# lucidrains/nuwa-pytorch

Hardware: AMD Instinct MI355X
Metric: video-tokens/sec, 3DNA decoder fwd+bwd @ 10x16x16 (higher is better)
Workload: dtype bf16/fp16 operands, fp32 accumulate -- forward: 3-MFMA bf16 hi+lo pairs on cross-attention kv projection, to_logits; 2 fp16 MFMAs (fp16 activation x fp16 hi+lo weight) on to_out x2, cross-attention q projection; single fp16 MFMA on 3DNA q/k/v projection, FF1 + gate, FF2, Sparse3DNA core, cross-atten

## Files before the change

nuwa_pytorch_amd/csrc/s3_args.h:

```cpp
#pragma once
#include "common.h"
#include "../../include/amdnuwa.h"

struct S3Args {
    const bf16_t *q, *k, *v, *ql, *kl, *vl; int ld;
    bf16_t *o, *ol; int ldo;
    int ol_f16;
    const bf16_t *dO, *dOl; int lddo;
    bf16_t *dq, *dk, *dv, *dql, *dkl, *dvl; int ldd;
    const float* wth;
    const float* bias;
    float *ds, *pm;
    float* stats;
    float *part_th, *part_k0, *part_v0;
    float* dwth;
    int B, ntok, F, H, W, kf, kh, kw, df, dh, dw, NH;
    int of, oh, ow;
    int xmode, FK, kvrows, kvoff, ldk, lddk;
    const bf16_t *k0, *k0l, *v0, *v0l; long long k0_bs;
    const uint8_t* kmask;
    float *dnull_k, *dnull_v;
    float scale;
    int accumulate;
    int dbg;
    int ymajor;
    int sep_passes;
    int packed;
    const float* gs2;
    int NT, TW, SW;
};

struct S3DropArgs : S3Args { const uint8_t* keep; float drop_s; };
template <bool DROP> struct S3KArgsSel { using type = S3Args; };
template <> struct S3KArgsSel<true> { using type = S3DropArgs; };
template <bool DROP> using S3KArgs = typename S3KArgsSel<DROP>::type;
template <bool DROP> inline S3KArgs<DROP> s3_kargs(const S3Args& a, const uint8_t* keep, float drop_s) {
    if constexpr (DROP) {
        S3DropArgs d{};
        static_cast<S3Args&>(d) = a;
        d.keep = keep; d.drop_s = drop_s;
        return d;
    } else {
        return a;
    }
}

struct S3Tile { int tw, nt, sw; };
inline S3Tile s3_tile(const amdnuwa_s3_geom* g) {
    if (g->W * g->heads * 4 <= 512) return {g->W, 1, g->W};
    const int twmax = 128 / g->heads, nt = (g->W + twmax - 1) / twmax, tw = (g->W + nt - 1) / nt;
    long long halo = (long long)(g->kw - 1) * g->dw;
    if (halo > 65536) halo = 65536;
    return {tw, nt, tw + (int)halo};
}
int s3w_fwd_launch(const S3Args& a, int dim_head, bool lo, size_t lds, const uint8_t* keep, float drop_s, hipStream_t stream);
int s3w_bwd_launch(const S3Args& a, int dim_head, bool lo, size_t lds_q, size_t lds_kv, const uint8_t* keep, float drop_s, hipStream_t stream);

namespace {

template <bool F16> __device__ __forceinline__ float ld16_t(bf16_t v) { return F16 ? (float)__builtin_bit_cast(_Float16, v) : bf2f(v); }

constexpr float NEG_MAX = -3.4028234663852886e38f;

__device__ __forceinline__ int xcd_row_id() {
    const int nb = gridDim.x, id = blockIdx.x, per = nb >> 3, rem = nb & 7, x = id & 7, k = id >> 3;
    return x * per + (x < rem ? x : rem) + k;
}
// ... 75 lines not shown
```

nuwa_pytorch_amd/csrc/sparse3dna.hip:

```cpp
#include <cmath>
#include "common.h"
#include "s3_args.h"

namespace {

constexpr int KHMAX = 3;

struct PlaneIt { int ta, tb, fr, yr; };

template <int CH, typename Fn>
__device__ __forceinline__ void sweep_taps(const S3Args& a, const bf16_t* src, const bf16_t* srcl, int b, int f, int y, int w,
                                           int h, int c, bool act, bool qvalid, bf16_t* st_hi, Fn&& fn) {
    const int HS = a.W * a.NH * 32;
    bf16_t* st_lo = st_hi + (CH / 8) * HS;
    const int myslot = ((w * a.NH + h) * 4 + c) * 8;
    const int yr0 = y - a.oh * a.dh;
    uint4 rh[CH / 8], rl[CH / 8];
    auto seek = [&](PlaneIt& p) {
        while (p.ta < a.kf && !(p.fr >= 0 && p.yr >= 0 && p.fr < a.FK && p.yr < a.H)) {
            ++p.tb; p.yr += a.dh;
            if (p.tb == a.kh) { p.tb = 0; p.yr = yr0; ++p.ta; p.fr += a.df; }
        }
    };
    auto step = [&](PlaneIt& p) {
// ... 468 lines not shown
                *reinterpret_cast<uint4*>(sq_hi + myslot + v8 * HS) = rq[v8];
                *reinterpret_cast<uint4*>(sd_hi + myslot + v8 * HS) = rd[v8];
                if (a.ql) *reinterpret_cast<uint4*>(sq_lo + myslot + v8 * HS) = rql[v8];
                if (a.dOl) *reinterpret_cast<uint4*>(sd_lo + myslot + v8 * HS) = rdl[v8];
            }
        }
        __syncthreads();
        float cds[KWMAX], cpm[KWMAX];
#pragma unroll
        for (int tc = 0; tc < KWMAX; ++tc) { cds[tc] = nds[tc]; cpm[tc] = npm[tc]; }
        const int tn = next_plane(tp + 1);
        if (tn < nplanes) fetch(tn);
        if (kvalid) {
            int fq, yq;
            plane(tp, fq, yq);
            for (int tc = 0; tc < a.kw; ++tc) {
                const int wq = w + (a.ow - tc) * a.dw;
                if (wq < 0 || wq >= a.W) continue;
                const int pq = (fq * a.H + yq) * a.W + wq;
                if (1 + pq >= a.ntok) continue;
                float dsv, pmv;
                if (tc < KWMAX) { dsv = tc == 0 ? cds[0] : (tc == 1 ? cds[1] : cds[2]); pmv = tc == 0 ? cpm[0] : (tc == 1 ? cpm[1] : cpm[2]); }
                else {
                    const size_t ci = (((size_t)b * nq + pq) * J + 1 + slot_plane(tp) * a.kw + tc) * a.NH + h;
                    dsv = a.ds[ci]; pmv = a.pm[ci];
                }
                const int slot = ((wq * a.NH + h) * 4 + c) * 8;
                if (LO) {
                    float qq[CH], dd[CH];
                    load_chunk<CH>(sq_hi + slot, a.ql ? sq_lo + slot : nullptr, qq, HS);
                    load_chunk<CH>(sd_hi + slot, a.dOl ? sd_lo + slot : nullptr, dd, HS);
#pragma unroll
                    for (int e = 0; e < CH; ++e) { dkf[e] += dsv * qq[e]; dvf[e] += pmv * dd[e]; }
                } else {
                    uint32_t qk2[CH / 2], dk2[CH / 2];
                    load_pk<CH>(sq_hi + slot, qk2, HS);
                    load_pk<CH>(sd_hi + slot, dk2, HS);
                    axpy_pk<CH>(dkf, dsv, qk2);
                    axpy_pk<CH>(dvf, pmv, dk2);
                }
            }
        }
        tp = tn;
    }
    if (kvalid) {
#pragma unroll
        for (int e = 0; e < CH; ++e) dkf[e] *= a.scale;
        const size_t g = ((size_t)b * a.kvrows + ik) * a.lddk + h * DH + c * CH;
        store_chunk<CH>(a.dk + g, a.dkl ? a.dkl + g : nullptr, dkf);
        store_chunk<CH>(a.dv + g, a.dvl ? a.dvl + g : nullptr, dvf);
    }
}

__global__ __launch_bounds__(1024) void s3_bwd_fin_kernel(S3Args a, int DH) {
    __shared__ float red[2][16][64];
    const int rows = a.F * a.H * a.NT, inner = a.NH * DH;
    const int lane = threadIdx.x & 63, rg = threadIdx.x >> 6;
    const int nchunk = (inner + 63) / 64;
    if ((int)blockIdx.x >= a.B * nchunk) {
        __shared__ float redw[64][17];
        const int nn = a.NH * a.NH;
        const int col = (blockIdx.x - a.B * nchunk) * 16 + (threadIdx.x & 15), rg64 = threadIdx.x >> 4;
        float s = 0.f;
        if (col < nn) {
            const int n = a.B * rows;
            for (int k = rg64; k < n; k += 64 * 8) {
                float v[8];
#pragma unroll
                for (int u = 0; u < 8; ++u) {
                    const int ku = k + 64 * u;
                    const float t = a.part_th[(size_t)(ku < n ? ku : 0) * nn + col];
                    v[u] = ku < n ? t : 0.f;
                }
#pragma unroll
                for (int u = 0; u < 8; ++u) s += v[u];
            }
        }
        redw[rg64][threadIdx.x & 15] = s;
        __syncthreads();
        if (rg64 == 0 && col < nn) {
            float t = 0.f;
#pragma unroll
            for (int r = 0; r < 64; ++r) t += redw[r][threadIdx.x & 15];
            t *= f16_gs_inv(a.gs2);
            a.dwth[col] = a.accumulate ? a.dwth[col] + t : t;
        }
        return;
    }
    if (a.xmode) {
        if ((int)blockIdx.x >= nchunk) return;
        const int e = blockIdx.x * 64 + lane;
        float sk = 0.f, sv = 0.f;
        if (e < inner)
            for (int r = rg; r < a.B * rows; r += 16) {
                sk += a.part_k0[(size_t)r * inner + e];
                sv += a.part_v0[(size_t)r * inner + e];
            }
        red[0][rg][lane] = sk;
        red[1][rg][lane] = sv;
        __syncthreads();
        if (rg == 0 && e < inner) {
            float tk = 0.f, tv = 0.f;
#pragma unroll
            for (int r = 0; r < 16; ++r) { tk += red[0][r][lane]; tv += red[1][r][lane]; }
            a.dnull_k[e] = tk;
            a.dnull_v[e] = tv;
        }
        return;
    }
    const int b = blockIdx.x / nchunk, e = (blockIdx.x % nchunk) * 64 + lane;
    float sk = 0.f, sv = 0.f;
    if (e < inner)
        for (int r = rg; r < rows; r += 16 * 4) {
            float vk[4], vv[4];
#pragma unroll
            for (int u = 0; u < 4; ++u) {
                const int ru = r + 16 * u;
                const size_t o = ((size_t)b * rows + (ru < rows ? ru : 0)) * inner + e;
                const float tk = a.part_k0[o], tv = a.part_v0[o];
                vk[u] = ru < rows ? tk : 0.f; vv[u] = ru < rows ? tv : 0.f;
            }
#pragma unroll
            for (int u = 0; u < 4; ++u) { sk += vk[u]; sv += vv[u]; }
        }
    red[0][rg][lane] = sk;
    red[1][rg][lane] = sv;
    __syncthreads();
    if (rg == 0 && e < inner) {
        float tk = 0.f, tv = 0.f;
#pragma unroll
        for (int r = 0; r < 16; ++r) { tk += red[0][r][lane]; tv += red[1][r][lane]; }
        const size_t gi = ((size_t)b * a.ntok) * a.lddo + e, go = ((size_t)b * a.ntok) * a.ldd + e;
        if (a.gs2) {
            tv += ld16_t<true>(a.dO[gi]);
            float amax = fmaxf(fabsf(tk), fabsf(tv));
            a.dk[go] = f2h_sat(tk); a.dv[go] = f2h_sat(tv);
            f16_sat_commit(amax);
            return;
        }
        tv += bf2f(a.dO[gi]) + (a.dOl ? bf2f(a.dOl[gi]) : 0.f);
        bf16_t hh, ll;
        f2bf_hilo(tk, hh, ll); a.dk[go] = hh; if (a.dkl) a.dkl[go] = ll;
        f2bf_hilo(tv, hh, ll); a.dv[go] = hh; if (a.dvl) a.dvl[go] = ll;
    }
}

int check_geom(const amdnuwa_s3_geom* g) {
    if (!g) return AMDNUWA_ERR_ARG;
    if (g->dim_head != 32 && g->dim_head != 64) return AMDNUWA_ERR_UNSUPPORTED;
    if (g->heads < 1 || g->heads > 8 || g->W < 1 || (g->W * g->heads * 4 > 512 && g->W > 64)) return AMDNUWA_ERR_UNSUPPORTED;
    if (g->kf < 1 || g->kh < 1 || g->kw < 1 || g->df < 1 || g->dh < 1 || g->dw < 1) return AMDNUWA_ERR_ARG;
    if (g->ntok < 1 || g->ntok - 1 > g->F * g->H * g->W) return AMDNUWA_ERR_ARG;
    return AMDNUWA_OK;
}
constexpr size_t S3_LDS_MAX = 160 * 1024 - 2048;
struct S3Lds { size_t fwd, bq, bkv; };
S3Lds s3_lds(const amdnuwa_s3_geom* g, bool lo) {
    const S3Tile tl = s3_tile(g);
    const size_t J = (size_t)g->kf * g->kh * g->kw + 1, inner = (size_t)g->heads * g->dim_head, tw = (size_t)tl.tw, sw = (size_t)tl.sw;
    const size_t stage = sw * inner * (lo ? 4 : 2), nsp = tw * J * g->heads;
    size_t spdp = 2 * nsp;
    if (spdp < tw * inner) spdp = tw * inner;
    return {stage + nsp * 4, stage + (spdp + 8 * 64) * 4, sw * inner * 8};
}
size_t s3_lds_need(const amdnuwa_s3_geom* g, bool lo) {
    const S3Lds l = s3_lds(g, lo);
    const size_t m = l.fwd > l.bq ? l.fwd : l.bq;
    return m > l.bkv ? m : l.bkv;
}
typedef __attribute__((address_space(3))) s16x4 lds_s16x4_t;
__device__ __forceinline__ int vt_off(int row, int gc) { return row * 128 + ((gc ^ (row & 7)) << 4); }
__device__ __forceinline__ bf16x8 vt_tr(const char* tile, int db, int c, int g4) {
    const int col = db * 16 + ((c & 3) << 2);
    const int r0 = 4 * g4 + (c >> 2), r1 = 16 + r0;
    const s16x4 lo = __builtin_amdgcn_ds_read_tr16_b64_v4i16((lds_s16x4_t*)(tile + vt_off(r0, col >> 3) + ((col >> 2) & 1) * 8));
    const s16x4 hi = __builtin_amdgcn_ds_read_tr16_b64_v4i16((lds_s16x4_t*)(tile + vt_off(r1, col >> 3) + ((col >> 2) & 1) * 8));
// ... 1025 lines not shown
#pragma unroll
            for (int i = 0; i < ROWS; ++i)
#pragma unroll
                for (int db = 0; db < 4; ++db) O[i][db] = f32x4{0.f, 0.f, 0.f, 0.f};
        }
#pragma unroll
        for (int i = 0; i < ROWS; ++i) {
            if (!r.qok[i]) continue;
            const size_t go = (r.tok0 + r.iq[i]) * a.ldo + g * DH + 4 * r.g4;
#pragma unroll
            for (int db = 0; db < 4; ++db) {
                const uint32_t h01 = pack2_rne(O[i][db][0], O[i][db][1]), h23 = pack2_rne(O[i][db][2], O[i][db][3]);
                if (!F16 || a.o) *reinterpret_cast<uint2*>(a.o + go + db * 16) = make_uint2(h01, h23);
                if (F16 && a.ol)
                    *reinterpret_cast<uint2*>(a.ol + go + db * 16) = a.ol_f16 ?
                        make_uint2(pack2_f16_sat(O[i][db][0], O[i][db][1]), pack2_f16_sat(O[i][db][2], O[i][db][3])) :
                        make_uint2(pack2_rne(O[i][db][0] - lo_f(h01), O[i][db][1] - hi_f(h01)), pack2_rne(O[i][db][2] - lo_f(h23), O[i][db][3] - hi_f(h23)));
            }
        }
    }
}

typedef _Float16 f16x4_t __attribute__((ext_vector_type(4)));
constexpr float S3Q_DPS = 0.015625f;
template <bool BIAS, bool G16 = false>
__global__ __launch_bounds__(512, 4) void s3_bwd_q_mfma_kernel(S3Args a) {
    constexpr int NH = S3M_NH, DH = S3M_DH, W = S3M_W, inner = NH * DH;
    extern __shared__ __attribute__((aligned(16))) char smem[];
    const int J = a.kf * a.kh * a.kw + 1, TS = s3m_ts(J), nsp = W * TS;
    const float rJ = 1.f / (float)J;
    const size_t r1 = (size_t)nsp * 4 > 8 * 4096 ? (size_t)nsp * 4 : 8 * 4096;
    float* SP = reinterpret_cast<float*>(smem);
    float* DP = reinterpret_cast<float*>(smem + r1);
    float* RED = DP + nsp;
    float* PM0 = RED + 8 * 64;
    __shared__ float wsh[64];
    __shared__ int pslot[S3M_PLANES + 1], ptok[S3M_PLANES + 1];
    const int t = threadIdx.x;
    const int rows = a.F * a.H;
    const int bid = xcd_row_id();
    const int b = bid / rows, r2 = bid % rows;
    int f, y;
    s3m_row_order(a, r2, f, y);
    const int ry = f * a.H + y;
    const int nq = a.ntok - 1;
    if (t < NH * NH) wsh[t] = a.wth[t];
    float* pth = a.part_th + (size_t)bid * NH * NH;
    float* pk0 = a.part_k0 + (size_t)bid * inner;
    float* pv0 = a.part_v0 + (size_t)bid * inner;
    if (ry == 0)
        for (int e = t; e < inner; e += blockDim.x) a.dq[((size_t)b * a.ntok) * a.ldd + e] = 0;
    if (ry * W + 1 >= a.ntok) {
        for (int e = t; e < NH * NH; e += blockDim.x) pth[e] = 0.f;
        for (int e = t; e < inner; e += blockDim.x) { pk0[e] = 0.f; pv0[e] = 0.f; }
        return;
    }
    {
        const float4 neg4 = make_float4(NEG_MAX, NEG_MAX, NEG_MAX, NEG_MAX), zero4 = make_float4(0.f, 0.f, 0.f, 0.f);
        for (int e = t; e < nsp / 4 && !(a.dbg & 2048); e += blockDim.x) { reinterpret_cast<float4*>(SP)[e] = neg4; reinterpret_cast<float4*>(DP)[e] = zero4; }
    }
    rowm_planes(a, f, y, pslot, ptok);
    const RowM r = rowm_init(a, b, ry, pslot, ptok);
    char* stile = reinterpret_cast<char*>(PM0 + W * NH) + r.wave * 2048;
    if (!(a.dbg & 1)) {
    if constexpr (!BIAS) {
    mfma_band_scores_fast<G16>(a, r, a.k, a.ld, a.q, a.ld, r.wave, SP, 1.f, stile);
    mfma_band_scores_fast<G16>(a, r, a.v, a.ld, a.dO, a.lddo, r.wave, DP, G16 ? S3Q_DPS : 1.f, stile);
    } else {
    mfma_band_scores_staged<G16>(a, r, a.k, a.ld, a.q, a.ld, r.wave, SP, BIAS ? a.scale : 1.f, BIAS ? a.bias : nullptr, stile);
    mfma_band_scores_staged<G16>(a, r, a.v, a.ld, a.dO, a.lddo, r.wave, DP, G16 ? S3Q_DPS : 1.f, nullptr, stile);
    }
    }
    __syncthreads();
    float* gst = a.stats ? a.stats + ((size_t)b * nq + (size_t)ry * W) * NH * 4 : nullptr;
    const int wvalid = a.ntok - 1 - ry * W;
    if (!(a.dbg & 64)) rowm_softmax(SP, J, gst, wvalid, BIAS ? 1.f : a.scale);
    __syncthreads();
    if constexpr (G16) {
        const int lane = t & 63, wv = t >> 6, n16 = lane & 15, kg = lane >> 4, sset = n16 >> 3, kh = kg & 1;
        const bool on = (n16 < 8) == (kg < 2);
        f16x4_t awt_hi, awt_lo;
#pragma unroll
        for (int i = 0; i < 4; ++i) {
            const float wt = on ? wsh[(4 * kh + i) * NH + (n16 & 7)] : 0.f;
            const _Float16 h16 = (_Float16)wt;
            awt_hi[i] = h16; awt_lo[i] = (_Float16)(wt - (float)h16);
        }
        const int nitems = W * J, ngrp = (nitems + 31) >> 5;
        f32x4 CW = {0.f, 0.f, 0.f, 0.f};
        float dp_amax = 0.f;
        for (int G = wv; G < ngrp && !(a.dbg & 128); G += 8) {
            {
                const int ib0 = 32 * G + 16 * sset + 4 * kg;
                float avf[4], bvf[4];
#pragma unroll
                for (int ts = 0; ts < 4; ++ts) {
                    const int item = ib0 + ((ts + sset + 2 * kh) & 3);
                    const bool ok = item < nitems;
                    const int idx = s3m_item(ok ? item : 0, rJ) + (n16 & 7);
                    avf[ts] = ok ? DP[idx] : 0.f;
                    bvf[ts] = ok ? SP[idx] : 0.f;
                }
                const f16x4_t av = __builtin_bit_cast(f16x4_t, make_uint2(pack2_f16_sat(avf[0], avf[1]), pack2_f16_sat(avf[2], avf[3])));
                const f16x4_t bv = __builtin_bit_cast(f16x4_t, make_uint2(pack2_f16(bvf[0], bvf[1]), pack2_f16(bvf[2], bvf[3])));
                CW = __builtin_amdgcn_mfma_f32_16x16x16f16(av, bv, CW, 0, 0, 0);
            }
            const int item = 32 * G + 16 * (kg >> 1) + n16;
// ... 236 lines not shown
            const float4 p4 = *reinterpret_cast<const float4*>(SP + ib);
            const float4 s4 = *reinterpret_cast<const float4*>(DP + ib);
            const f16x4_t pf = __builtin_bit_cast(f16x4_t, ok ? make_uint2(pack2_f16(p4.x, p4.y), pack2_f16(p4.z, p4.w)) : make_uint2(0u, 0u));
            f32x4 pm = {0.f, 0.f, 0.f, 0.f};
            pm = __builtin_amdgcn_mfma_f32_16x16x16f16(aw_hi, pf, pm, 0, 0, 0);
            pm = __builtin_amdgcn_mfma_f32_16x16x16f16(aw_lo, pf, pm, 0, 0, 0);
            if (ok && j == 0) {
#pragma unroll
                for (int i = 0; i < 4; ++i) PM0[wq * NH + 4 * kh + i] = iq < a.ntok ? pm[i] : 0.f;
            }
            if (ok && iq < a.ntok && keep && !(a.dbg & 2)) {
                uint4* dst = reinterpret_cast<uint4*>(reinterpret_cast<uint32_t*>(a.pm) + (((size_t)b * nq + (iq - 1)) * J + j) * NH + 4 * kh);
                *dst = make_uint4(pack2_f16(s4.x, pm[0]), pack2_f16(s4.y, pm[1]), pack2_f16(s4.z, pm[2]), pack2_f16(s4.w, pm[3]));
            }
        }
        __syncthreads();
    } else if (a.packed) {
        const float* wv = wsh;
        const int ta0 = max(0, a.kf - 1 - f / a.df), tb0 = max(0, a.kh - 1 - y / a.dh);
        const float rkw = 1.f / (float)a.kw, rkh = 1.f / (float)a.kh;
        for (int item = t; item < W * J && !(a.dbg & 512); item += blockDim.x) {
            const int wq = (int)(((float)item + 0.5f) * rJ), j = item - wq * J;
            const int iq = 1 + ry * W + wq;
            bool keep = false;
            if (j > 0) {
                const int pl = (int)(((float)(j - 1) + 0.5f) * rkw), tc = j - 1 - pl * a.kw;
                const int ta = (int)(((float)pl + 0.5f) * rkh), tb = pl - ta * a.kh;
                keep = ta >= ta0 && tb >= tb0 && wq - (a.kw - 1 - tc) * a.dw >= 0;
            }
            const int ib = item * NH + wq * S3M_PAD;
            const float4 p0 = *reinterpret_cast<const float4*>(SP + ib), p1 = *reinterpret_cast<const float4*>(SP + ib + 4);
            const float4 s0 = *reinterpret_cast<const float4*>(DP + ib), s1 = *reinterpret_cast<const float4*>(DP + ib + 4);
            const float pv[8] = {p0.x, p0.y, p0.z, p0.w, p1.x, p1.y, p1.z, p1.w};
            const float dsv[8] = {s0.x, s0.y, s0.z, s0.w, s1.x, s1.y, s1.z, s1.w};
            uint32_t pw[8];
#pragma unroll
            for (int g = 0; g < 8; ++g) {
                const float4 w0 = *reinterpret_cast<const float4*>(wv + g * NH), w1 = *reinterpret_cast<const float4*>(wv + g * NH + 4);
                const float wg[8] = {w0.x, w0.y, w0.z, w0.w, w1.x, w1.y, w1.z, w1.w};
                float sm = 0.f;
#pragma unroll
                for (int hh = 0; hh < 8; ++hh) sm += wg[hh] * pv[hh];
                if (j == 0) PM0[wq * NH + g] = iq < a.ntok ? sm : 0.f;
                pw[g] = pack2_t<G16>(dsv[g], sm);
            }
            if (iq < a.ntok && keep && !gst && !(a.dbg & 2)) {
                uint4* dst = reinterpret_cast<uint4*>(reinterpret_cast<uint32_t*>(a.pm) + (((size_t)b * nq + (iq - 1)) * J + j) * NH);
                dst[0] = make_uint4(pw[0], pw[1], pw[2], pw[3]);
                dst[1] = make_uint4(pw[4], pw[5], pw[6], pw[7]);
            }
        }
        __syncthreads();
    }
    {
        const int h = r.wave;
        f32x4 O[4] = {f32x4{0.f, 0.f, 0.f, 0.f}, f32x4{0.f, 0.f, 0.f, 0.f}, f32x4{0.f, 0.f, 0.f, 0.f}, f32x4{0.f, 0.f, 0.f, 0.f}};
        if (!(a.dbg & 4)) mfma_band_apply_fast<G16>(a, r, a.k, a.ld, h, DP, smem + r.wave * 4096, O);
        if (r.qok) {
            bf16_t* orow = a.dq + (r.tok0 + r.iq) * a.ldd + h * DH + 4 * r.g4;
            float amax = 0.f;
#pragma unroll
            for (int db = 0; db < 4; ++db)
                *reinterpret_cast<uint2*>(orow + db * 16) = G16 ?
                    make_uint2(pack2_f16_sat_n(O[db][0] * a.scale, O[db][1] * a.scale, amax), pack2_f16_sat_n(O[db][2] * a.scale, O[db][3] * a.scale, amax)) :
                    make_uint2(pack2_rne(O[db][0] * a.scale, O[db][1] * a.scale), pack2_rne(O[db][2] * a.scale, O[db][3] * a.scale));
            if constexpr (G16) f16_sat_commit(amax);
        }
    }
    __syncthreads();
    if (!(a.dbg & 1024)) {
        float* part = reinterpret_cast<float*>(smem);
        const int eg = t & 63, wv = t >> 6, h = eg >> 3;
        float sk[8], sv[8];
#pragma unroll
        for (int k = 0; k < 8; ++k) { sk[k] = 0.f; sv[k] = 0.f; }
        uint4 qv[2], dv4[2];
        float cs[2], cp[2];
#pragma unroll
        for (int rr = 0; rr < 2; ++rr) {
            const int w = 2 * wv + rr, i = 1 + ry * W + w;
            const bool in = i < a.ntok;
            const size_t ic = r.tok0 + (in ? i : a.ntok - 1);
            qv[rr] = *reinterpret_cast<const uint4*>(a.q + ic * a.ld + 8 * eg);
            dv4[rr] = *reinterpret_cast<const uint4*>(a.dO + ic * a.lddo + 8 * eg);
            cs[rr] = in ? DP[w * TS + h] : 0.f;
            cp[rr] = in ? PM0[w * NH + h] : 0.f;
        }
#pragma unroll
        for (int rr = 0; rr < 2; ++rr) {
            const uint32_t qw[4] = {qv[rr].x, qv[rr].y, qv[rr].z, qv[rr].w}, dw[4] = {dv4[rr].x, dv4[rr].y, dv4[rr].z, dv4[rr].w};
#pragma unroll
            for (int k = 0; k < 4; ++k) {
                sk[2 * k] = fmaf(cs[rr], lo_t<G16>(qw[k]), sk[2 * k]); sk[2 * k + 1] = fmaf(cs[rr], hi_t<G16>(qw[k]), sk[2 * k + 1]);
                sv[2 * k] = fmaf(cp[rr], lo_t<G16>(dw[k]), sv[2 * k]); sv[2 * k + 1] = fmaf(cp[rr], hi_t<G16>(dw[k]), sv[2 * k + 1]);
            }
        }
        float4* dst = reinterpret_cast<float4*>(part + (wv * 64 + eg) * 16);
        const int rot = eg >> 2;
        dst[rot & 3] = make_float4(sk[0], sk[1], sk[2], sk[3]); dst[(1 + rot) & 3] = make_float4(sk[4], sk[5], sk[6], sk[7]);
        dst[(2 + rot) & 3] = make_float4(sv[0], sv[1], sv[2], sv[3]); dst[(3 + rot) & 3] = make_float4(sv[4], sv[5], sv[6], sv[7]);
    }
    __syncthreads();
    if (!(a.dbg & 1024)) {
        const float* part = reinterpret_cast<const float*>(smem);
        for (int e = t; e < inner; e += blockDim.x) {
            const int eg = e >> 3, cmp = e & 7, rot = eg >> 2;
            const int ok_ = 4 * (((cmp >> 2) + rot) & 3) + (cmp & 3), ov_ = 4 * ((2 + (cmp >> 2) + rot) & 3) + (cmp & 3);
            float sk = 0.f, sv = 0.f;
#pragma unroll
            for (int wv = 0; wv < 8; ++wv) {
                sk += part[(wv * 64 + eg) * 16 + ok_];
                sv += part[(wv * 64 + eg) * 16 + ov_];
            }
            pk0[e] = a.scale * sk;
            pv0[e] = sv;
        }
    }
}

template <bool PACKED, bool G16 = false>
__global__ __launch_bounds__(512, 2) void s3_bwd_kv_mfma_kernel(S3Args a) {
    constexpr int NH = S3M_NH, DH = S3M_DH, W = S3M_W;
    extern __shared__ __attribute__((aligned(16))) char smem[];
    __shared__ int pslot[S3M_PLANES + 1], ptok[S3M_PLANES + 1];
    const int t = threadIdx.x, lane = t & 63, wave = t >> 6, c = lane & 15, g4 = lane >> 4, h = wave;
    const int rows = a.F * a.H;
    const int bid = xcd_row_id();
    const int b = bid / rows, r2 = bid % rows;
    int f, y;
    s3m_row_order(a, r2, f, y);
    const int ry = f * a.H + y;
    const int J = a.kf * a.kh * a.kw + 1, nq = a.ntok - 1;
    if (ry * W + 1 >= a.ntok) return;
    if (t < 64) {
        const int ta = t / a.kh, tb = t % a.kh;
        const int fq = f + (a.kf - 1 - ta) * a.df, yq = y + (a.kh - 1 - tb) * a.dh;
        const bool ok = t < a.kf * a.kh && fq < a.F && yq < a.H && (fq * a.H + yq) * W + 1 < a.ntok;
        const unsigned long long m = __ballot(ok);
        if (ok) {
            const int pos = __popcll(m & ((1ull << t) - 1ull));
            pslot[pos] = 1 + (ta * a.kh + tb) * a.kw; ptok[pos] = 1 + (fq * a.H + yq) * W;
        }
        if (t == 0) pslot[S3M_PLANES] = __popcll(m);
    }
    __syncthreads();
    const int nplanes = pslot[S3M_PLANES];
    const size_t tok0 = (size_t)b * a.ntok;
    int tsel[4];
#pragma unroll
    for (int j = 0; j < 4; ++j) {
        const int d = (4 * g4 + j) - c;
        tsel[j] = -1;
#pragma unroll
        for (int tc = 0; tc < S3M_KW; ++tc)
            if (tc < a.kw && d == (a.kw - 1 - tc) * a.dw) tsel[j] = tc;
    }
    char* tq = smem + wave * 8192;
    char* td = tq + 4096;
    const int gc = lane & 7, r8 = lane >> 3;
    const bf16_t* qbase = a.q + tok0 * a.ld + h * DH + gc * 8;
    const bf16_t* dbase = a.dO + tok0 * a.lddo + h * DH + gc * 8;
    int woff[4], troff[4];
#pragma unroll
    for (int i = 0; i < 4; ++i) woff[i] = vt_off(r8 + 8 * i, gc);
    {
        const int r0 = 4 * g4 + (c >> 2);
#pragma unroll
        for (int db = 0; db < 4; ++db) {
            const int col = db * 16 + ((c & 3) << 2);
            troff[db] = vt_off(r0, col >> 3) + ((col >> 2) & 1) * 8;
        }
    }
    uint4 sq[4], sd[4];
    float cs[8], cp[8];
    uint32_t cw[8];
    const int vps = lane < nplanes ? pslot[lane] : 0, vpt = lane < nplanes ? ptok[lane] : 0;
    const int hu = __builtin_amdgcn_readfirstlane(h);
    const char* sbq = reinterpret_cast<const char*>(a.q + tok0 * a.ld + hu * DH);
    const char* sbd = reinterpret_cast<const char*>(a.dO + tok0 * a.lddo + hu * DH);
    const char* sbw = reinterpret_cast<const char*>(reinterpret_cast<const uint32_t*>(a.pm) + (size_t)b * nq * J * NH + hu);
    const unsigned ldqb = (unsigned)a.ld * 2u, lddb = (unsigned)a.lddo * 2u;
    const unsigned vq0 = (unsigned)r8 * ldqb + (unsigned)gc * 16u, vq1 = vq0 + 8u * ldqb;
    const unsigned vd0 = (unsigned)r8 * lddb + (unsigned)gc * 16u, vd1 = vd0 + 8u * lddb;
    unsigned cj[4];
#pragma unroll
    for (int j = 0; j < 4; ++j) cj[j] = 32u * (unsigned)((4 * g4 + j) * J + (tsel[j] < 0 ? 0 : tsel[j]));
    auto fetch = [&](int pi) {
        if constexpr (PACKED) {
#pragma unroll
            for (int kb = 0; kb < 2; ++kb) {
                const int pj = pi + kb;
                if (pj >= nplanes) {
                    sq[2 * kb] = sq[2 * kb + 1] = sd[2 * kb] = sd[2 * kb + 1] = make_uint4(0, 0, 0, 0);
#pragma unroll
                    for (int j = 0; j < 4; ++j) cw[kb * 4 + j] = 0u;
                    continue;
                }
                const int base = __builtin_amdgcn_readlane(vpt, pj < 64 ? pj : 63);
                const unsigned soq = (unsigned)base * ldqb, sod = (unsigned)base * lddb;
                const unsigned sw = 32u * (unsigned)((base - 1) * J + __builtin_amdgcn_readlane(vps, pj < 64 ? pj : 63));
                const bool nof = (a.dbg & 32) != 0, nog = (a.dbg & 16) != 0;
                if (base + 16 <= a.ntok && !nof && !nog) {
                    sq[2 * kb] = ldg_u4(sbq, soq + vq0); sq[2 * kb + 1] = ldg_u4(sbq, soq + vq1);
                    sd[2 * kb] = ldg_u4(sbd, sod + vd0); sd[2 * kb + 1] = ldg_u4(sbd, sod + vd1);
#pragma unroll
                    for (int j = 0; j < 4; ++j) cw[kb * 4 + j] = tsel[j] >= 0 ? *reinterpret_cast<const uint32_t*>(sbw + (sw + cj[j])) : 0u;
                } else {
                    const bool ok0 = base + r8 < a.ntok && !nof, ok1 = base + r8 + 8 < a.ntok && !nof;
// ... 36 lines not shown
    f32x4 dK[4], dV[4];
#pragma unroll
    for (int db = 0; db < 4; ++db) dK[db] = dV[db] = f32x4{0.f, 0.f, 0.f, 0.f};
    if (nplanes > 0) fetch(0);
    for (int pi = 0; pi < nplanes; pi += 2) {
#pragma unroll
        for (int i = 0; i < 4; ++i) {
            *reinterpret_cast<uint4*>(tq + woff[i]) = sq[i];
            *reinterpret_cast<uint4*>(td + woff[i]) = sd[i];
        }
        bf16x8 bs, bp;
        if constexpr (PACKED) {
            bs = __builtin_bit_cast(bf16x8, make_uint4(__builtin_amdgcn_perm(cw[1], cw[0], 0x05040100u), __builtin_amdgcn_perm(cw[3], cw[2], 0x05040100u),
                                                       __builtin_amdgcn_perm(cw[5], cw[4], 0x05040100u), __builtin_amdgcn_perm(cw[7], cw[6], 0x05040100u)));
            bp = __builtin_bit_cast(bf16x8, make_uint4(__builtin_amdgcn_perm(cw[1], cw[0], 0x07060302u), __builtin_amdgcn_perm(cw[3], cw[2], 0x07060302u),
                                                       __builtin_amdgcn_perm(cw[5], cw[4], 0x07060302u), __builtin_amdgcn_perm(cw[7], cw[6], 0x07060302u)));
        } else {
            bs = __builtin_bit_cast(bf16x8, make_uint4(pack2_rne(cs[0], cs[1]), pack2_rne(cs[2], cs[3]), pack2_rne(cs[4], cs[5]), pack2_rne(cs[6], cs[7])));
            bp = __builtin_bit_cast(bf16x8, make_uint4(pack2_rne(cp[0], cp[1]), pack2_rne(cp[2], cp[3]), pack2_rne(cp[4], cp[5]), pack2_rne(cp[6], cp[7])));
        }
        if (pi + 2 < nplanes) fetch(pi + 2);
        __builtin_amdgcn_wave_barrier();
#pragma unroll
        for (int db = 0; db < 4; ++db) {
            const s16x4 ql = __builtin_amdgcn_ds_read_tr16_b64_v4i16((lds_s16x4_t*)(tq + troff[db]));
            const s16x4 qh = __builtin_amdgcn_ds_read_tr16_b64_v4i16((lds_s16x4_t*)(tq + troff[db] + 2048));
            const s16x4 dl = __builtin_amdgcn_ds_read_tr16_b64_v4i16((lds_s16x4_t*)(td + troff[db]));
            const s16x4 dh_ = __builtin_amdgcn_ds_read_tr16_b64_v4i16((lds_s16x4_t*)(td + troff[db] + 2048));
            const s16x8 q8 = {ql[0], ql[1], ql[2], ql[3], qh[0], qh[1], qh[2], qh[3]};
            const s16x8 d8 = {dl[0], dl[1], dl[2], dl[3], dh_[0], dh_[1], dh_[2], dh_[3]};
            dK[db] = mfma16<G16>(__builtin_bit_cast(bf16x8, q8), bs, dK[db]);
            dV[db] = mfma16<G16>(__builtin_bit_cast(bf16x8, d8), bp, dV[db]);
        }
        __builtin_amdgcn_wave_barrier();
    }
    const int ik = 1 + ry * W + c;
    if (ik < a.ntok) {
        bf16_t* kr = a.dk + (tok0 + ik) * a.ldd + h * DH + 4 * g4;
        bf16_t* vr = a.dv + (tok0 + ik) * a.ldd + h * DH + 4 * g4;
        float amax = 0.f;
#pragma unroll
        for (int db = 0; db < 4; ++db) {
            if constexpr (G16) {
                *reinterpret_cast<uint2*>(kr + db * 16) = make_uint2(pack2_f16_sat_n(dK[db][0] * a.scale, dK[db][1] * a.scale, amax),
                                                                     pack2_f16_sat_n(dK[db][2] * a.scale, dK[db][3] * a.scale, amax));
                *reinterpret_cast<uint2*>(vr + db * 16) = make_uint2(pack2_f16_sat_n(dV[db][0], dV[db][1], amax), pack2_f16_sat_n(dV[db][2], dV[db][3], amax));
            } else {
                *reinterpret_cast<uint2*>(kr + db * 16) = make_uint2(pack2_rne(dK[db][0] * a.scale, dK[db][1] * a.scale),
                                                                     pack2_rne(dK[db][2] * a.scale, dK[db][3] * a.scale));
                *reinterpret_cast<uint2*>(vr + db * 16) = make_uint2(pack2_rne(dV[db][0], dV[db][1]), pack2_rne(dV[db][2], dV[db][3]));
            }
        }
        if constexpr (G16) f16_sat_commit(amax);
    }
}

__global__ __launch_bounds__(512, 2) void s3_bwd_kv_rc_mfma_kernel(S3Args a) {
    constexpr int NH = S3M_NH, DH = S3M_DH, W = S3M_W;
    constexpr bool G16 = false;
    extern __shared__ __attribute__((aligned(16))) char smem[];
    __shared__ int pslot[S3M_PLANES + 1], ptok[S3M_PLANES + 1];
    __shared__ float wsh[64];
    const int t = threadIdx.x, lane = t & 63, wave = t >> 6, c = lane & 15, g4 = lane >> 4, h = wave;
    const int rows = a.F * a.H;
    const int bid = xcd_row_id();
    const int b = bid / rows, r2 = bid % rows;
    int f, y;
    s3m_row_order(a, r2, f, y);
    const int ry = f * a.H + y;
    const int nq = a.ntok - 1;
    if (ry * W + 1 >= a.ntok) return;
    if (t < NH * NH) wsh[t] = a.wth[t];
    if (t == 0) {
        int n = 0;
        for (int ta = 0; ta < a.kf; ++ta)
            for (int tb = 0; tb < a.kh; ++tb) {
                const int fq = f + (a.kf - 1 - ta) * a.df, yq = y + (a.kh - 1 - tb) * a.dh;
                if (fq < a.F && yq < a.H && (fq * a.H + yq) * W + 1 < a.ntok) {
                    pslot[n] = 1 + (ta * a.kh + tb) * a.kw; ptok[n] = 1 + (fq * a.H + yq) * W; ++n;
                }
            }
        pslot[S3M_PLANES] = n;
    }
    __syncthreads();
    const int nplanes = pslot[S3M_PLANES];
    const size_t tok0 = (size_t)b * a.ntok;
    int tsel[4];
#pragma unroll
    for (int j = 0; j < 4; ++j) {
        const int d = (4 * g4 + j) - c;
        tsel[j] = -1;
#pragma unroll
        for (int tc = 0; tc < S3M_KW; ++tc)
            if (tc < a.kw && d == (a.kw - 1 - tc) * a.dw) tsel[j] = tc;
    }
    const int ik = 1 + ry * W + c;
    const bool kok = ik < a.ntok;
    const bf16_t* krow = a.k + (tok0 + (kok ? ik : 0)) * a.ld + h * DH + g4 * 8;
    const bf16_t* vrow = a.v + (tok0 + (kok ? ik : 0)) * a.ld + h * DH + g4 * 8;
    const bf16x8 kf0 = ldg8(krow, kok), kf1 = ldg8(krow + 32, kok), vf0 = ldg8(vrow, kok), vf1 = ldg8(vrow + 32, kok);
    float wg[8], wt[8];
#pragma unroll
    for (int e = 0; e < 8; ++e) {
        wg[e] = __builtin_bit_cast(float, __builtin_amdgcn_readfirstlane(__builtin_bit_cast(int, wsh[h * NH + e])));
        wt[e] = __builtin_bit_cast(float, __builtin_amdgcn_readfirstlane(__builtin_bit_cast(int, wsh[e * NH + h])));
    }
// ... 271 lines not shown
extern "C" int amdnuwa_s3_supported(const amdnuwa_s3_geom* g, int lo_operands) {
    if (check_geom(g)) return 0;
    return s3_lds_need(g, lo_operands != 0) <= S3_LDS_MAX ? 1 : 0;
}

extern "C" size_t amdnuwa_sparse3dna_bwd_workspace_bytes(const amdnuwa_s3_geom* g) {
    if (check_geom(g)) return 0;
    const size_t J = (size_t)g->kf * g->kh * g->kw + 1, nq = g->ntok - 1, rows = (size_t)g->B * g->F * g->H * s3_tile(g).nt;
    const size_t inner = (size_t)g->heads * g->dim_head;
    return (2 * (size_t)g->B * nq * J * g->heads + rows * g->heads * g->heads + 2 * rows * inner) * sizeof(float) + 256 +
           amdnuwa_colsum_workspace_bytes((long long)g->B * nq, (int)(J * g->heads));
}

static int s3_bwd_run(const amdnuwa_s3_geom* g, const uint16_t* q, const uint16_t* k, const uint16_t* v,
                      const uint16_t* q_lo, const uint16_t* k_lo, const uint16_t* v_lo, int ld,
                      const float* w_th, const uint16_t* dO, const uint16_t* dO_lo, int lddo,
                      uint16_t* dq, uint16_t* dk, uint16_t* dv, uint16_t* dq_lo, uint16_t* dk_lo,
                      uint16_t* dv_lo, int ldd, float* dw_th, int accumulate, void* workspace,
                      size_t workspace_bytes, const uint8_t* keep, float drop_s, hipStream_t stream) {
    int rc = check_geom(g);
    if (rc) return rc;
    if (s3_lds_need(g, k_lo != nullptr) > S3_LDS_MAX) return AMDNUWA_ERR_UNSUPPORTED;
    if (!q || !k || !v || !w_th || !dO || !dq || !dk || !dv || !dw_th || ld % 8 || lddo % 8 || ldd % 8) return AMDNUWA_ERR_ARG;
    if (!workspace || workspace_bytes < amdnuwa_sparse3dna_bwd_workspace_bytes(g)) return AMDNUWA_ERR_WORKSPACE;
    if (g->B <= 0) return AMDNUWA_OK;
    S3Args a{};
    fill_geom(a, g);
    a.q = q; a.k = k; a.v = v; a.ql = q_lo; a.kl = k_lo; a.vl = v_lo; a.ld = ld; a.wth = w_th;
    a.dO = dO; a.dOl = dO_lo; a.lddo = lddo;
    a.dq = dq; a.dk = dk; a.dv = dv; a.dql = dq_lo; a.dkl = dk_lo; a.dvl = dv_lo; a.ldd = ldd;
    a.dwth = dw_th; a.accumulate = accumulate;
    a.dbg = g_amdnuwa_tuning[17];
    a.sep_passes = g_amdnuwa_tuning[19] == 1;
    self_kv(a);
    const size_t J = (size_t)g->kf * g->kh * g->kw + 1, nq = g->ntok - 1, rows = (size_t)g->B * g->F * g->H;
    const size_t inner = (size_t)g->heads * g->dim_head;
    float* ws = (float*)workspace;
    a.ds = ws; ws += (size_t)g->B * nq * J * g->heads;
    a.pm = ws; ws += (size_t)g->B * nq * J * g->heads;
    const size_t parts = rows * a.NT;
    a.part_th = ws; ws += parts * g->heads * g->heads;
    a.part_k0 = ws; ws += parts * inner;
    a.part_v0 = ws;
    const bool has_lo = k_lo != nullptr;
    if (has_lo && (!q_lo || !v_lo)) return AMDNUWA_ERR_ARG;
    const S3Lds l = s3_lds(g, has_lo);
    const size_t lds_q = l.bq, lds_kv = l.bkv;
    dim3 grid((unsigned)rows), block(block_threads(g));
    const bool q_mfma = !keep && !has_lo && !dO_lo && !g->noncausal && g_amdnuwa_tuning[4] != 1 && g->W == 16 && g->heads == 8 && g->dim_head == 64 &&
                        g->kw <= S3M_KW && g->kf * g->kh <= S3M_PLANES && ld % 8 == 0 && lddo % 8 == 0 && ldd % 4 == 0;
    const bool kv_rc = q_mfma && g_amdnuwa_tuning[4] == 4 && !g->d_rel_bias;
    a.stats = kv_rc ? a.ds : nullptr;
    a.packed = (q_mfma && g_amdnuwa_tuning[4] != 2 && !g->d_rel_bias && g_amdnuwa_tuning[24] != 1 && !a.sep_passes) ? 1 : 0;
    const size_t nspm = (size_t)g->W * (J * g->heads + 4);
    const size_t lds_qm = (nspm * 4 > 8 * 4096 ? nspm * 4 : 8 * 4096) + nspm * 4 + (8 * 64 + 16 * 8) * 4 + 8 * 2048;
#define S3B(DH_, LO_, DR_)                                                                                        \
    do {                                                                                                          \
        if (q_mfma && a.bias) {                                                                                   \
            (void)hipFuncSetAttribute((const void*)s3_bwd_q_mfma_kernel<true>, hipFuncAttributeMaxDynamicSharedMemorySize, (int)lds_qm); \
            hipLaunchKernelGGL(s3_bwd_q_mfma_kernel<true>, grid, dim3(512), lds_qm, stream, a);                   \
        } else if (q_mfma) {                                                                                      \
            (void)hipFuncSetAttribute((const void*)s3_bwd_q_mfma_kernel<false>, hipFuncAttributeMaxDynamicSharedMemorySize, (int)lds_qm); \
            hipLaunchKernelGGL(s3_bwd_q_mfma_kernel<false>, grid, dim3(512), lds_qm, stream, a);                  \
        } else {                                                                                                  \
            (void)hipFuncSetAttribute((const void*)s3_bwd_q_kernel<DH_, LO_, DR_>, hipFuncAttributeMaxDynamicSharedMemorySize, (int)lds_q); \
            hipLaunchKernelGGL((s3_bwd_q_kernel<DH_, LO_, DR_>), grid, block, lds_q, stream, s3_kargs<DR_>(a, keep, drop_s)); \
        }                                                                                                         \
        LAUNCH_CHECK();                                                                                           \
        if (kv_rc) {                                                                                              \
            (void)hipFuncSetAttribute((const void*)s3_bwd_kv_rc_mfma_kernel, hipFuncAttributeMaxDynamicSharedMemorySize, 8 * 4096 + 16384); \
            hipLaunchKernelGGL(s3_bwd_kv_rc_mfma_kernel, grid, dim3(512), 8 * 4096 + 16384, stream, a);           \
        } else if (q_mfma && g_amdnuwa_tuning[4] != 2 && a.packed) {                                              \
            (void)hipFuncSetAttribute((const void*)s3_bwd_kv_mfma_kernel<true>, hipFuncAttributeMaxDynamicSharedMemorySize, 8 * 8192); \
            hipLaunchKernelGGL(s3_bwd_kv_mfma_kernel<true>, grid, dim3(512), 8 * 8192, stream, a);                \
        } else if (q_mfma && g_amdnuwa_tuning[4] != 2) {                                                          \
            (void)hipFuncSetAttribute((const void*)s3_bwd_kv_mfma_kernel<false>, hipFuncAttributeMaxDynamicSharedMemorySize, 8 * 8192); \
            hipLaunchKernelGGL(s3_bwd_kv_mfma_kernel<false>, grid, dim3(512), 8 * 8192, stream, a);               \
        } else {                                                                                                  \
            (void)hipFuncSetAttribute((const void*)s3_bwd_kv_kernel<DH_, LO_>, hipFuncAttributeMaxDynamicSharedMemorySize, (int)lds_kv); \
            hipLaunchKernelGGL((s3_bwd_kv_kernel<DH_, LO_>), grid, block, lds_kv, stream, a);                     \
        }                                                                                                         \
    } while (0)
    const bool lo_mode = has_lo || dO_lo != nullptr;
    if (lo_mode && (!has_lo || !dO_lo)) return AMDNUWA_ERR_ARG;
    if (a.NT > 1) {
        const int rcw = s3w_bwd_launch(a, g->dim_head, lo_mode, lds_q, lds_kv, keep, drop_s, stream);
        if (rcw) return rcw;
    } else if (keep) {
        if (g->dim_head == 64) { if (lo_mode) S3B(64, true, true); else S3B(64, false, true); }
        else { if (lo_mode) S3B(32, true, true); else S3B(32, false, true); }
    } else if (g->dim_head == 64) { if (lo_mode) S3B(64, true, false); else S3B(64, false, false); }
    else { if (lo_mode) S3B(32, true, false); else S3B(32, false, false); }
#undef S3B
    LAUNCH_CHECK();
    hipLaunchKernelGGL(s3_bwd_fin_kernel, dim3(g->B * (((int)inner + 63) / 64) + (g->heads * g->heads + 15) / 16), dim3(1024), 0, stream, a, g->dim_head);
    LAUNCH_CHECK();
    if (g->d_rel_bias) {
        float* cws = a.part_v0 + parts * inner;
        const int rc2 = amdnuwa_colsum(a.ds, g->d_rel_bias, (long long)g->B * nq, (int)(J * g->heads), 0, cws,
                                       amdnuwa_colsum_workspace_bytes((long long)g->B * nq, (int)(J * g->heads)), stream);
        if (rc2) return rc2;
    }
    return AMDNUWA_OK;
}

extern "C" int amdnuwa_sparse3dna_bwd(const amdnuwa_s3_geom* g, const uint16_t* q, const uint16_t* k, const uint16_t* v,
                                      const uint16_t* q_lo, const uint16_t* k_lo, const uint16_t* v_lo, int ld,
                                      const float* w_th, const uint16_t* dO, const uint16_t* dO_lo, int lddo,
                                      uint16_t* dq, uint16_t* dk, uint16_t* dv, uint16_t* dq_lo, uint16_t* dk_lo,
                                      uint16_t* dv_lo, int ldd, float* dw_th, int accumulate, void* workspace,
                                      size_t workspace_bytes, hipStream_t stream) {
    return s3_bwd_run(g, q, k, v, q_lo, k_lo, v_lo, ld, w_th, dO, dO_lo, lddo, dq, dk, dv, dq_lo, dk_lo, dv_lo, ldd, dw_th, accumulate,
                      workspace, workspace_bytes, nullptr, 1.f, stream);
}

extern "C" int amdnuwa_sparse3dna_bwd_drop(const amdnuwa_s3_geom* g, const uint16_t* q, const uint16_t* k, const uint16_t* v,
                                           const uint16_t* q_lo, const uint16_t* k_lo, const uint16_t* v_lo, int ld,
                                           const float* w_th, const uint16_t* dO, const uint16_t* dO_lo, int lddo,
                                           uint16_t* dq, uint16_t* dk, uint16_t* dv, uint16_t* dq_lo, uint16_t* dk_lo,
                                           uint16_t* dv_lo, int ldd, float* dw_th, int accumulate, void* workspace,
                                           size_t workspace_bytes, const uint8_t* keep, float drop_scale, hipStream_t stream) {
    const int rc = drop_geom(g, k_lo != nullptr);
    if (rc) return rc;
    if (!drop_args_ok(keep, drop_scale)) return AMDNUWA_ERR_ARG;
    return s3_bwd_run(g, q, k, v, q_lo, k_lo, v_lo, ld, w_th, dO, dO_lo, lddo, dq, dk, dv, dq_lo, dk_lo, dv_lo, ldd, dw_th, accumulate,
                      workspace, workspace_bytes, keep, drop_scale, stream);
}

extern "C" int amdnuwa_sparse3dna_bwd_f16_supported(const amdnuwa_s3_geom* g) {
    return check_geom(g) == AMDNUWA_OK && s3_mfma_geom(g) && !g->rel_bias && !g->d_rel_bias ? 1 : 0;
}
extern "C" int amdnuwa_sparse3dna_bwd_f16(const amdnuwa_s3_geom* g, const uint16_t* q_f16, const uint16_t* k_f16, const uint16_t* v_f16, int ld,
                                          const float* w_th, const uint16_t* dO_f16, int lddo, uint16_t* dq_f16, uint16_t* dk_f16,
                                          uint16_t* dv_f16, int ldd, float* dw_th, int accumulate, const float* scale2, void* workspace,
                                          size_t workspace_bytes, hipStream_t stream) {
    int rc = check_geom(g);
    if (rc) return rc;
    if (!amdnuwa_sparse3dna_bwd_f16_supported(g)) return AMDNUWA_ERR_UNSUPPORTED;
    if (!q_f16 || !k_f16 || !v_f16 || !w_th || !dO_f16 || !dq_f16 || !dk_f16 || !dv_f16 || !dw_th || !scale2 || ld % 8 || lddo % 8 || ldd % 8)
        return AMDNUWA_ERR_ARG;
    if (!workspace || workspace_bytes < amdnuwa_sparse3dna_bwd_workspace_bytes(g)) return AMDNUWA_ERR_WORKSPACE;
    if (g->B <= 0) return AMDNUWA_OK;
    S3Args a{};
    fill_geom(a, g);
    a.q = q_f16; a.k = k_f16; a.v = v_f16; a.ld = ld; a.wth = w_th;
    a.dO = dO_f16; a.lddo = lddo;
    a.dq = dq_f16; a.dk = dk_f16; a.dv = dv_f16; a.ldd = ldd;
    a.dwth = dw_th; a.accumulate = accumulate; a.gs2 = scale2;
    a.dbg = g_amdnuwa_tuning[17];
    self_kv(a);
    const size_t J = (size_t)g->kf * g->kh * g->kw + 1, nq = g->ntok - 1, rows = (size_t)g->B * g->F * g->H;
    const size_t inner = (size_t)g->heads * g->dim_head;
    float* ws = (float*)workspace;
    a.ds = ws; ws += (size_t)g->B * nq * J * g->heads;
    a.pm = ws; ws += (size_t)g->B * nq * J * g->heads;
    a.part_th = ws; ws += rows * g->heads * g->heads;
    a.part_k0 = ws; ws += rows * inner;
    a.part_v0 = ws;
    a.packed = 1;
    const size_t nspm = (size_t)g->W * (J * g->heads + 4);
    const size_t lds_qm = (nspm * 4 > 8 * 4096 ? nspm * 4 : 8 * 4096) + nspm * 4 + (8 * 64 + 16 * 8) * 4 + 8 * 2048;
    const dim3 grid((unsigned)rows);
    (void)hipFuncSetAttribute((const void*)s3_bwd_q_mfma_kernel<false, true>, hipFuncAttributeMaxDynamicSharedMemorySize, (int)lds_qm);
    hipLaunchKernelGGL((s3_bwd_q_mfma_kernel<false, true>), grid, dim3(512), lds_qm, stream, a);
    LAUNCH_CHECK();
    (void)hipFuncSetAttribute((const void*)s3_bwd_kv_mfma_kernel<true, true>, hipFuncAttributeMaxDynamicSharedMemorySize, 8 * 8192);
    hipLaunchKernelGGL((s3_bwd_kv_mfma_kernel<true, true>), grid, dim3(512), 8 * 8192, stream, a);
    LAUNCH_CHECK();
    hipLaunchKernelGGL(s3_bwd_fin_kernel, dim3(g->B * (((int)inner + 63) / 64) + (g->heads * g->heads + 15) / 16), dim3(1024), 0, stream, a, g->dim_head);
    LAUNCH_CHECK();
    return AMDNUWA_OK;
}

namespace {
int cross_setup(S3Args& a, const amdnuwa_s3_geom* g, int ctx_rows, const uint16_t* k, const uint16_t* v, const uint16_t* k_lo,
                const uint16_t* v_lo, int ldkv, const uint16_t* null_k, const uint16_t* null_k_lo, const uint16_t* null_v,
                const uint16_t* null_v_lo, const uint8_t* key_mask) {
    int rc = check_geom(g);
    if (rc) return rc;
    if (s3_lds_need(g, k_lo != nullptr) > S3_LDS_MAX) return AMDNUWA_ERR_UNSUPPORTED;
    if (!k || !v || !null_k || !null_v || ldkv % 8) return AMDNUWA_ERR_ARG;
    if (g->rel_bias || ctx_rows != g->kf * g->H * g->W) return AMDNUWA_ERR_ARG;
    if ((k_lo != nullptr) != (v_lo != nullptr) || (k_lo != nullptr) != (null_k_lo != nullptr) || (k_lo != nullptr) != (null_v_lo != nullptr))
        return AMDNUWA_ERR_ARG;
    fill_geom(a, g);
    a.xmode = 1; a.FK = g->kf; a.kvrows = ctx_rows; a.kvoff = 0; a.kmask = key_mask;
    a.of = 0; a.df = 1;
    a.oh = (g->kh - 1) / 2; a.ow = (g->kw - 1) / 2;
    a.k = k; a.v = v; a.kl = k_lo; a.vl = v_lo; a.ldk = ldkv;
    a.k0 = null_k; a.k0l = null_k_lo; a.v0 = null_v; a.v0l = null_v_lo; a.k0_bs = 0;
    return AMDNUWA_OK;
}
}

extern "C" int amdnuwa_cross2dna_fwd(const amdnuwa_s3_geom* g, const uint16_t* q, const uint16_t* q_lo, int ldq, int ctx_rows,
                                     const uint16_t* k, const uint16_t* v, const uint16_t* k_lo, const uint16_t* v_lo, int ldkv,
                                     const uint16_t* null_k, const uint16_t* null_k_lo, const uint16_t* null_v,
                                     const uint16_t* null_v_lo, const uint8_t* key_mask, const float* w_th, uint16_t* o,
                                     uint16_t* o_lo, int ldo, hipStream_t stream) {
    S3Args a{};
    int rc = cross_setup(a, g, ctx_rows, k, v, k_lo, v_lo, ldkv, null_k, null_k_lo, null_v, null_v_lo, key_mask);
    if (rc) return rc;
    if (!q || !w_th || !o || ldq % 8 || ldo % 8 || (k_lo != nullptr) != (q_lo != nullptr)) return AMDNUWA_ERR_ARG;
    if (g->B <= 0) return AMDNUWA_OK;
    a.q = q; a.ql = q_lo; a.ld = ldq; a.o = o; a.ol = o_lo; a.ldo = ldo; a.wth = w_th;
    const bool lo_mode = k_lo != nullptr;
    const size_t lds = s3_lds(g, lo_mode).fwd;
    if (a.NT > 1) return s3w_fwd_launch(a, g->dim_head, lo_mode, lds, nullptr, 1.f, stream);
    dim3 grid(g->B * g->F * g->H), block(block_threads(g));
#define S3F(DH_, LO_)                                                                                             \
    do {                                                                                                          \
        (void)hipFuncSetAttribute((const void*)s3_fwd_kernel<DH_, LO_>, hipFuncAttributeMaxDynamicSharedMemorySize, (int)lds); \
// ... 65 lines not shown
```

Measured before the change: 713,100.

## Move BOS key/value gradient partials from q-backward into kv-backward kernel

```diff
diff --git a/nuwa_pytorch_amd/csrc/s3_args.h b/nuwa_pytorch_amd/csrc/s3_args.h
--- a/nuwa_pytorch_amd/csrc/s3_args.h
+++ b/nuwa_pytorch_amd/csrc/s3_args.h
@@ -13,6 +13,7 @@
     float *ds, *pm;
     float* stats;
     float *part_th, *part_k0, *part_v0;
+    float* bos_c;
     float* dwth;
     int B, ntok, F, H, W, kf, kh, kw, df, dh, dw, NH;
     int of, oh, ow;
diff --git a/nuwa_pytorch_amd/csrc/sparse3dna.hip b/nuwa_pytorch_amd/csrc/sparse3dna.hip
--- a/nuwa_pytorch_amd/csrc/sparse3dna.hip
+++ b/nuwa_pytorch_amd/csrc/sparse3dna.hip
@@ -544,35 +544,36 @@
     }
 }
 
-__global__ __launch_bounds__(1024) void s3_bwd_fin_kernel(S3Args a, int DH) {
+__global__ __launch_bounds__(1024, 8) void s3_bwd_fin_kernel(S3Args a, int DH) {
     __shared__ float red[2][16][64];
     const int rows = a.F * a.H * a.NT, inner = a.NH * DH;
     const int lane = threadIdx.x & 63, rg = threadIdx.x >> 6;
-    const int nchunk = (inner + 63) / 64;
-    if ((int)blockIdx.x >= a.B * nchunk) {
+    const int nchunk = (inner + 63) / 64, nwb = (a.NH * a.NH + 15) / 16, bidx = (int)blockIdx.x - nwb;
+    if (bidx < 0) {
         __shared__ float redw[64][17];
         const int nn = a.NH * a.NH;
-        const int col = (blockIdx.x - a.B * nchunk) * 16 + (threadIdx.x & 15), rg64 = threadIdx.x >> 4;
+        const int col = blockIdx.x * 16 + (threadIdx.x & 15), rg64 = threadIdx.x >> 4;
         float s = 0.f;
         if (col < nn) {
             const int n = a.B * rows;
-            for (int k = rg64; k < n; k += 64 * 8) {
-                float v[8];
-#pragma unroll
-                for (int u = 0; u < 8; ++u) {
-                    const int ku = k + 64 * u;
-                    const float t = a.part_th[(size_t)(ku < n ? ku : 0) * nn + col];
-                    v[u] = ku < n ? t : 0.f;
+            const unsigned loff = (unsigned)(rg64 * nn + col);
+            for (int k0 = 0; k0 < n; k0 += 64 * 32) {
+                float v[32];
+#pragma unroll
+                for (int u = 0; u < 32; ++u) {
+                    const int kb = k0 + 64 * u;
+                    v[u] = 0.f;
+                    if (kb + rg64 < n) v[u] = (a.part_th + (size_t)kb * nn)[loff];
                 }
 #pragma unroll
-                for (int u = 0; u < 8; ++u) s += v[u];
+                for (int u = 0; u < 32; ++u) s += v[u];
             }
         }
         redw[rg64][threadIdx.x & 15] = s;
         __syncthreads();
         if (rg64 == 0 && col < nn) {
             float t = 0.f;
-#pragma unroll
+#pragma unroll 16
             for (int r = 0; r < 64; ++r) t += redw[r][threadIdx.x & 15];
             t *= f16_gs_inv(a.gs2);
             a.dwth[col] = a.accumulate ? a.dwth[col] + t : t;
@@ -580,8 +581,8 @@
         return;
     }
     if (a.xmode) {
-        if ((int)blockIdx.x >= nchunk) return;
-        const int e = blockIdx.x * 64 + lane;
+        if (bidx >= nchunk) return;
+        const int e = bidx * 64 + lane;
         float sk = 0.f, sv = 0.f;
         if (e < inner)
             for (int r = rg; r < a.B * rows; r += 16) {
@@ -600,20 +601,22 @@
         }
         return;
     }
-    const int b = blockIdx.x / nchunk, e = (blockIdx.x % nchunk) * 64 + lane;
+    const int b = bidx / nchunk, e = (bidx % nchunk) * 64 + lane;
+    const int rgu = __builtin_amdgcn_readfirstlane(rg);
+    const float* bk = a.part_k0 + (size_t)b * rows * inner;
+    const float* bv = a.part_v0 + (size_t)b * rows * inner;
     float sk = 0.f, sv = 0.f;
     if (e < inner)
-        for (int r = rg; r < rows; r += 16 * 4) {
-            float vk[4], vv[4];
-#pragma unroll
-            for (int u = 0; u < 4; ++u) {
+        for (int r = rgu; r < rows; r += 16 * 12) {
+            float vk[12], vv[12];
+#pragma unroll
+            for (int u = 0; u < 12; ++u) {
                 const int ru = r + 16 * u;
-                const size_t o = ((size_t)b * rows + (ru < rows ? ru : 0)) * inner + e;
-                const float tk = a.part_k0[o], tv = a.part_v0[o];
-                vk[u] = ru < rows ? tk : 0.f; vv[u] = ru < rows ? tv : 0.f;
-            }
-#pragma unroll
-            for (int u = 0; u < 4; ++u) { sk += vk[u]; sv += vv[u]; }
+                vk[u] = 0.f; vv[u] = 0.f;
+                if (ru < rows) { vk[u] = (bk + (size_t)ru * inner)[e]; vv[u] = (bv + (size_t)ru * inner)[e]; }
+            }
+#pragma unroll
+            for (int u = 0; u < 12; ++u) { sk += vk[u]; sv += vv[u]; }
         }
     red[0][rg][lane] = sk;
     red[1][rg][lane] = sv;
@@ -1745,7 +1748,7 @@
         for (int e = t; e < inner; e += blockDim.x) a.dq[((size_t)b * a.ntok) * a.ldd + e] = 0;
     if (ry * W + 1 >= a.ntok) {
         for (int e = t; e < NH * NH; e += blockDim.x) pth[e] = 0.f;
-        for (int e = t; e < inner; e += blockDim.x) { pk0[e] = 0.f; pv0[e] = 0.f; }
+        for (int e = t; e < inner && !a.bos_c; e += blockDim.x) { pk0[e] = 0.f; pv0[e] = 0.f; }
         return;
     }
     {
@@ -2088,6 +2091,11 @@
         }
         __syncthreads();
     }
+    if (a.bos_c && t < W * NH) {
+        const int w = t >> 3, hh = t & 7;
+        if (w < wvalid)
+            reinterpret_cast<float2*>(a.bos_c)[((size_t)b * nq + (size_t)ry * W + w) * NH + hh] = make_float2(DP[w * TS + hh], PM0[w * NH + hh]);
+    }
     {
         const int h = r.wave;
         f32x4 O[4] = {f32x4{0.f, 0.f, 0.f, 0.f}, f32x4{0.f, 0.f, 0.f, 0.f}, f32x4{0.f, 0.f, 0.f, 0.f}, f32x4{0.f, 0.f, 0.f, 0.f}};
@@ -2103,6 +2111,7 @@
             if constexpr (G16) f16_sat_commit(amax);
         }
     }
+    if (a.bos_c) return;
     __syncthreads();
     if (!(a.dbg & 1024)) {
         float* part = reinterpret_cast<float*>(smem);
@@ -2167,7 +2176,10 @@
     s3m_row_order(a, r2, f, y);
     const int ry = f * a.H + y;
     const int J = a.kf * a.kh * a.kw + 1, nq = a.ntok - 1;
-    if (ry * W + 1 >= a.ntok) return;
+    if (ry * W + 1 >= a.ntok) {
+        if (a.bos_c) { a.part_k0[(size_t)bid * (NH * DH) + t] = 0.f; a.part_v0[(size_t)bid * (NH * DH) + t] = 0.f; }
+        return;
+    }
     if (t < 64) {
         const int ta = t / a.kh, tb = t % a.kh;
         const int fq = f + (a.kf - 1 - ta) * a.df, yq = y + (a.kh - 1 - tb) * a.dh;
@@ -2190,6 +2202,11 @@
 #pragma unroll
         for (int tc = 0; tc < S3M_KW; ++tc)
             if (tc < a.kw && d == (a.kw - 1 - tc) * a.dw) tsel[j] = tc;
+    }
+    float bcs = 0.f, bcp = 0.f;
+    if (a.bos_c && lane < W && lane < a.ntok - 1 - ry * W) {
+        const float2 cc = reinterpret_cast<const float2*>(a.bos_c)[((size_t)b * nq + (size_t)ry * W + lane) * NH + h];
+        bcs = cc.x; bcp = cc.y;
     }
     char* tq = smem + wave * 8192;
     char* td = tq + 4096;
@@ -2332,6 +2349,27 @@
             }
         }
         if constexpr (G16) f16_sat_commit(amax);
+    }
+    if (a.bos_c && !(a.dbg & 1024)) {
+        const int kb16 = ((nplanes - 1) & 1) * 16, gcl = lane >> 3, sub = (lane & 7) * 2;
+        const int ics = __builtin_bit_cast(int, bcs), icp = __builtin_bit_cast(int, bcp);
+        float sk = 0.f, sv = 0.f;
+#pragma unroll
+        for (int v = 0; v < 8; ++v) {
+            float pk = 0.f, pv = 0.f;
+#pragma unroll
+            for (int rr = 0; rr < 2; ++rr) {
+                const int w = 2 * v + rr;
+                const float cs0 = __builtin_bit_cast(float, __builtin_amdgcn_readlane(ics, w));
+                const float cp0 = __builtin_bit_cast(float, __builtin_amdgcn_readlane(icp, w));
+                const int off = vt_off(kb16 + w, gcl) + sub;
+                pk = fmaf(cs0, lo_t<G16>((uint32_t)*reinterpret_cast<const bf16_t*>(tq + off)), pk);
+                pv = fmaf(cp0, lo_t<G16>((uint32_t)*reinterpret_cast<const bf16_t*>(td + off)), pv);
+            }
+            sk += pk; sv += pv;
+        }
+        a.part_k0[(size_t)bid * (NH * DH) + t] = a.scale * sk;
+        a.part_v0[(size_t)bid * (NH * DH) + t] = sv;
     }
 }
 
@@ -2709,6 +2747,7 @@
     const bool kv_rc = q_mfma && g_amdnuwa_tuning[4] == 4 && !g->d_rel_bias;
     a.stats = kv_rc ? a.ds : nullptr;
     a.packed = (q_mfma && g_amdnuwa_tuning[4] != 2 && !g->d_rel_bias && g_amdnuwa_tuning[24] != 1 && !a.sep_passes) ? 1 : 0;
+    a.bos_c = (a.packed && !kv_rc && !a.bias && g_amdnuwa_tuning[26] != 1) ? a.ds : nullptr;
     const size_t nspm = (size_t)g->W * (J * g->heads + 4);
     const size_t lds_qm = (nspm * 4 > 8 * 4096 ? nspm * 4 : 8 * 4096) + nspm * 4 + (8 * 64 + 16 * 8) * 4 + 8 * 2048;
 #define S3B(DH_, LO_, DR_)                                                                                        \
@@ -2815,6 +2854,7 @@
     a.part_k0 = ws; ws += rows * inner;
     a.part_v0 = ws;
     a.packed = 1;
+    a.bos_c = g_amdnuwa_tuning[26] != 1 ? a.ds : nullptr;
     const size_t nspm = (size_t)g->W * (J * g->heads + 4);
     const size_t lds_qm = (nspm * 4 > 8 * 4096 ? nspm * 4 : 8 * 4096) + nspm * 4 + (8 * 64 + 16 * 8) * 4 + 8 * 2048;
     const dim3 grid((unsigned)rows);
```

After: 714,700, median of 6. About the same (+0.2%).
